# ikmb/vcf2prot

Hardware: AMD Instinct MI355X
Metric: amino-acids written/sec (higher is better)
Workload: dtype u8

## Files before the change

vcf2prot_amd/_native.py:

```python
from __future__ import annotations

import ctypes
import os
from ctypes import POINTER, c_char_p, c_double, c_int, c_int64, c_size_t, c_uint8, c_uint32, c_uint64, c_void_p

_PKG = os.path.dirname(os.path.abspath(__file__))
HIP_LIB_PATH = os.path.join(_PKG, "lib", "libvcf2prot_hip.so")
COHORT_LIB_PATH = os.path.join(_PKG, "lib", "libv2p_cohort.so")

V2P_OK = 0
ERR_NAMES = {
    0: "V2P_OK", -1: "V2P_ERR_INVALID_ARG", -2: "V2P_ERR_HIP", -3: "V2P_ERR_BAD_CODE", -4: "V2P_ERR_RES_OOB",
    -5: "V2P_ERR_SRC_OOB", -6: "V2P_ERR_NOT_CONTIGUOUS", -7: "V2P_ERR_NOT_CANONICAL", -8: "V2P_ERR_NON_BYTE_CHAR",
    -9: "V2P_ERR_UNSUPPORTED", -10: "V2P_ERR_STATE",
}
V2P_ERR_INVALID_ARG, V2P_ERR_HIP, V2P_ERR_BAD_CODE, V2P_ERR_RES_OOB, V2P_ERR_SRC_OOB = -1, -2, -3, -4, -5
V2P_ERR_NOT_CONTIGUOUS, V2P_ERR_NOT_CANONICAL, V2P_ERR_NON_BYTE_CHAR, V2P_ERR_UNSUPPORTED, V2P_ERR_STATE = -6, -7, -8, -9, -10
V2P_FLAG_DEBUG_GPU, V2P_FLAG_TEMPORAL, V2P_FLAG_RESULT_ORDER = 1, 2, 4


class v2p_chunk(ctypes.Structure):
    _fields_ = [("task_begin", c_uint64), ("dst_n", c_uint64)]


# ... 123 lines not shown

def hip_lib():
    global _hip
    if _hip is None:
        if not os.path.exists(HIP_LIB_PATH):
            raise RuntimeError(
                f"{HIP_LIB_PATH} is missing: build it with `python -m vcf2prot_amd.build` "
                "(the gpu engine has no CPU fallback)")
        _hip = _bind(ctypes.CDLL(HIP_LIB_PATH), HIP_API)
    return _hip


BENCH_LIB_PATH = os.path.join(_PKG, "lib", "libv2p_bench.so")
BENCH_API = {
    "v2p_copy_prefetch_launch": (c_int, [c_void_p, c_void_p, c_uint64, c_uint32, c_void_p, c_uint64, c_int, c_int, c_uint32]),
    "v2p_copy_mix_launch": (c_int, [c_void_p, c_void_p, c_uint64, c_uint32, c_void_p, c_uint64, c_void_p, c_uint32, c_uint32, c_uint32, c_uint32]),
    "v2p_copy_bench_launch": (c_int, [c_void_p, c_void_p, c_uint64, c_uint32, c_void_p, c_uint64, c_int, c_void_p]),
    "v2p_gather_bench_launch": (c_int, [c_void_p, c_void_p, c_uint64, c_uint32, c_uint32, c_uint32, c_void_p]),
    "v2p_fill_launch": (c_int, [c_void_p, c_void_p, c_uint64, c_uint32, c_int]),
    "v2p_stitch_launch": (c_int, [c_void_p, c_void_p, c_uint64, c_void_p, c_uint32, c_void_p, c_uint64, c_void_p, c_uint64,
                                  c_void_p, c_uint64, c_void_p, c_int, c_uint32]),
    "v2p_batch_download_patch_image": (c_int, [c_void_p, c_void_p, c_void_p, c_void_p, POINTER(c_uint64), POINTER(c_uint64)]),
    "v2p_bench_set_variant": (c_int, [c_void_p, c_uint32]),
    "v2p_scan_launch": (c_int, [c_void_p, c_int, c_void_p, c_uint64, c_void_p, c_void_p]),
}
_bench = None


def bench_lib():
    global _bench
    if _bench is None:
        if not os.path.exists(BENCH_LIB_PATH):
            from . import build
            build.build_bench()
        _bench = _bind(_bind(ctypes.CDLL(BENCH_LIB_PATH), HIP_API), BENCH_API)
    return _bench


def cohort_lib():
    global _cohort
    if _cohort is None:
        if not os.path.exists(COHORT_LIB_PATH):
            raise RuntimeError(f"{COHORT_LIB_PATH} is missing: build it with `python -m vcf2prot_amd.build`")
        from ._cohort_api import COHORT_API
        _cohort = _bind(ctypes.CDLL(COHORT_LIB_PATH), COHORT_API)
    return _cohort
# ... 9 lines not shown
```

vcf2prot_amd/csrc/stitch_device.hpp:

```cpp
#pragma once
#include <hip/hip_runtime.h>
#include <stdint.h>
#include "stitch_kernels.h"
#include "block_scan.hpp"

namespace v2p {

typedef uint32_t u32x4 __attribute__((ext_vector_type(4)));
struct __attribute__((packed, aligned(1))) unaligned16 { u32x4 v; };

__device__ __forceinline__ u32x4 gather16(uint64_t addr)
{
    typedef const __attribute__((address_space(1))) unaligned16* gptr;
    return reinterpret_cast<gptr>(addr)->v;
}

struct __attribute__((packed, aligned(4))) dwaligned16 { u32x4 v; };
__device__ __forceinline__ u32x4 gather16_dw(uint64_t addr)
{
    typedef const __attribute__((address_space(1))) dwaligned16* gptr;
    typedef const __attribute__((address_space(1))) uint32_t* dptr;
    const uint64_t base = addr & ~3ull;
    const uint32_t sh = uint32_t(addr) & 3u;
    const u32x4 v = reinterpret_cast<gptr>(base)->v;
// ... 42 lines not shown
    else if (q < 8) { lo = x; hi = y; }
    else { lo = 0ull; hi = x; }
    return u32x4{uint32_t(lo), uint32_t(lo >> 32), uint32_t(hi), uint32_t(hi >> 32)};
}

constexpr uint64_t ADJ_IMM = 1ull << 63;
constexpr uint64_t ADJ_LIT = (1ull << 40) - 1;

__device__ __forceinline__ void report(unsigned long long* status, uint64_t index, uint32_t reason)
{
    atomicMin(status, (unsigned long long)((index << 8) | reason));
}

__device__ __forceinline__ void lds_barrier()
{
    asm volatile("s_waitcnt lgkmcnt(0)" ::: "memory");
    __builtin_amdgcn_s_barrier();
    asm volatile("" ::: "memory");
}


__device__ __forceinline__ uint32_t touch_wave_first(uint32_t r, uint32_t q) { return r + 8u * 4u * q; }
__host__ __device__ __forceinline__ uint32_t touch_waves_per_xcd(uint32_t n_chunks) { return ((n_chunks + 7u) / 8u + 3u) / 4u; }
constexpr uint32_t STAGE_SLOTS = 64;
constexpr uint32_t TOUCH_CHUNKS_PER_WAVE = 4;
__device__ __forceinline__ void touch_chunks(const uint64_t* __restrict__ desc, const Chunk* __restrict__ chunks, uint32_t c0, uint32_t n_chunks, uint64_t n_desc,
                                             const uint8_t* __restrict__ payload, uint64_t payload_len, uint32_t lane, uint64_t* __restrict__ stage = nullptr,
                                             const uint64_t* __restrict__ rows = nullptr)
{
    if (c0 >= n_chunks) return;
    auto payload_lines = [&](uint64_t dd) {
        const uint64_t src = dd & SRC_MASK, len = (dd >> 40) & LEN_MASK;
        if ((dd >> 62) == SPACE_PAYLOAD && len != 0u && src < payload_len && len <= payload_len - src) {
            const uint32_t b0 = payload[src], b1 = payload[src + len - 1u];
            asm volatile("" :: "v"(b0), "v"(b1));
        }
    };
    if (rows) {
        uint64_t r[TOUCH_CHUNKS_PER_WAVE], t[TOUCH_CHUNKS_PER_WAVE];
#pragma unroll
        for (uint32_t k = 0; k < TOUCH_CHUNKS_PER_WAVE; ++k) {
            const uint32_t c = c0 + 8u * k < n_chunks ? c0 + 8u * k : c0;
            r[k] = rows[uint64_t(c) * STAGE_SLOTS + lane];
            t[k] = reinterpret_cast<const uint64_t*>(chunks + c)[lane & 1u];
        }
#pragma unroll
// ... 34 lines not shown
```

vcf2prot_amd/csrc/stitch_kernels.h:

```cpp
#pragma once
#include <hip/hip_runtime.h>
#include <stdint.h>
#include "sir_pack.hpp"

namespace v2p {

enum : uint32_t {
    STATUS_BAD_CODE = 1,
    STATUS_RES_OOB = 2,
    STATUS_SRC_OOB = 3,
    STATUS_NOT_CONTIGUOUS = 4
};
constexpr unsigned long long STATUS_CLEAN = ~0ull;
constexpr int STITCH_TASKS_PER_LANE = 4;
constexpr uint32_t DOTS_BYTES = 64u * 1024u + 128u;

struct StitchArgs {
    const uint64_t* desc;
    uint64_t        n_desc;
    const Chunk*    chunks;
    uint32_t        n_chunks;
    const uint8_t*  src0;
    uint64_t        src0_len;
    const uint8_t*  src1;
// ... 2 lines not shown
    uint64_t        out_len;
    unsigned long long* status;
    const uint8_t*  dots;
    const Chunk*    next_chunks = nullptr;
    uint32_t        n_next = 0;
    uint32_t        store_sc1 = 0;
    uint64_t        opt_phase_bytes = 0;
    uint32_t        opt_phase_min_chunks = 0;
    int32_t         opt_store_sc1 = -1;
    uint32_t        opt_touch = 0;
    uint32_t        opt_wave_bodies = 0;
    uint32_t        rows = 0;
    uint64_t        img_desc = 0, img_bytes = 0;
    hipStream_t     aux_stream = nullptr;
    hipEvent_t      ev_fork = nullptr, ev_join = nullptr;
    uint32_t        opt_dual = 0;
    uint64_t*       stage = nullptr;
    uint32_t        stage_chunks = 0;
    const uint64_t* stage_cur = nullptr;
    uint64_t*       stage_next = nullptr;
    const uint64_t* resident = nullptr;
    const uint64_t* rows_next = nullptr;
    uint32_t        phase_chunks = 0;
};

uint32_t stitch_stage_chunks(const StitchArgs& args, int nontemporal);
hipError_t launch_stage_rows(const StitchArgs& args, uint64_t* rows, hipStream_t stream);

struct OrderedArgs {
    const uint8_t*  code;
    const uint64_t* start_pos;
    const uint64_t* length;
    const uint64_t* start_pos_res;
    uint64_t        n_tasks;
    const uint8_t*  ref;
    const uint8_t*  alt;
    uint8_t*        res;
    uint64_t        esize;
};

struct ValidateArgs {
    const uint8_t*  code;
    const uint64_t* start_pos;
    const uint64_t* length;
    const uint64_t* start_pos_res;
    uint64_t        n_tasks;
    uint64_t        n_ref, n_alt, n_res;
// ... 25 lines not shown
```

vcf2prot_amd/csrc/stitch_kernels.hip:

```cpp
#include <hip/hip_runtime.h>
#include <utility>
#include <vector>
#include <stdint.h>
#include <stdlib.h>
#include <mutex>
#include "stitch_kernels.h"
#include "stitch_device.hpp"

namespace v2p {

__device__ __forceinline__ u32x4 overwrite_tail(u32x4 v, u32x4 ld, uint32_t ja, bool take)
{
    const uint64_t x = ~0ull << (8u * (ja & 7u));
    const uint64_t mlo = (take && ja < 8u) ? x : 0ull;
    const uint64_t mhi = take ? (ja < 8u ? ~0ull : x) : 0ull;
    const uint32_t k0 = uint32_t(mlo), k1 = uint32_t(mlo >> 32), k2 = uint32_t(mhi), k3 = uint32_t(mhi >> 32);
    v[0] = (v[0] & ~k0) | (ld[0] & k0);
    v[1] = (v[1] & ~k1) | (ld[1] & k1);
    v[2] = (v[2] & ~k2) | (ld[2] & k2);
    v[3] = (v[3] & ~k3) | (ld[3] & k3);
    return v;
}

template <bool DW>
// ... 1041 lines not shown
{
    if (blockIdx.x < n) rows[(first + blockIdx.x) * STAGE_SLOTS + threadIdx.x] = uint64_t(SPACE_FILL) << 62;
}

hipError_t launch_stage_rows(const StitchArgs& a, uint64_t* rows, hipStream_t stream)
{
    if (a.n_chunks == 0 || !rows) return hipSuccess;
    hipLaunchKernelGGL(touch_image_kernel, dim3(8u * ((touch_waves_per_xcd(a.n_chunks) + 3u) / 4u)), dim3(256), 0, stream, a.desc, a.chunks, a.n_chunks, a.n_desc, a.src1, a.src1_len, rows, nullptr);
    const uint32_t pad = (8u - (a.n_chunks & 7u)) & 7u;
    if (pad) hipLaunchKernelGGL(fill_rows_kernel, dim3(pad), dim3(64), 0, stream, rows, uint64_t(a.n_chunks), pad);
    return hipGetLastError();
}

static hipError_t launch_stitch_range(const StitchArgs& args, hipStream_t stream, int nontemporal, uint32_t max_blocks);

#ifdef V2P_BENCH_VARIANTS
__global__ void idle_kernel(uint32_t us)
{
    const uint64_t t0 = __builtin_readcyclecounter();
    while (__builtin_readcyclecounter() - t0 < uint64_t(us) * 100u) __builtin_amdgcn_s_sleep(64);
}
#endif

static uint64_t phase_plan(const StitchArgs& a, int nontemporal, uint32_t max_blocks, bool staged, bool* ride_out)
{
    *ride_out = false;
    if (a.n_chunks == 0) return 0;
    const uint64_t img_desc = a.img_desc ? a.img_desc : a.n_desc, img_bytes = a.img_bytes ? a.img_bytes : a.out_len;
    const bool rich = image_is_rich(img_desc, img_bytes);
    uint64_t phase_bytes = rich ? PHASE_BYTES_RICH : PHASE_BYTES_DEFAULT;
    if (staged && rich && a.src0_len <= PHASE_STAGED_SMALL_REF) phase_bytes = PHASE_BYTES_STAGED;
    if (a.opt_phase_bytes == ~0ull) phase_bytes = 0;
    else if (a.opt_phase_bytes != 0) phase_bytes = a.opt_phase_bytes;
    const bool streams = (nontemporal & 4) != 0 || (nontemporal & 16) == 0;
    const uint32_t min_chunks = a.opt_phase_min_chunks ? a.opt_phase_min_chunks : PHASE_MIN_CHUNKS;
    if (max_blocks != 0 || phase_bytes == 0 || !streams || a.n_chunks < min_chunks) return 0;
    const double per_chunk = 16.0 + 8.0 * double(img_desc) / double(a.n_chunks);
    uint64_t per = uint64_t(double(phase_bytes) / per_chunk);
    const uint64_t per_min = a.opt_phase_min_chunks ? 8u : 4096u;
    per = per < per_min ? per_min : (per & ~7ull);
    const bool no_touch = (a.opt_touch & 1u) != 0, own_touch = (a.opt_touch & 2u) != 0;
    *ride_out = !own_touch && !no_touch && (nontemporal & 4) != 0 && (nontemporal & 48) == 48 && !(nontemporal & 2);
    return per;
}

uint32_t stitch_stage_chunks(const StitchArgs& args, int nontemporal)
{
    bool ride = false;
    const uint64_t per = phase_plan(args, nontemporal, 0, true, &ride);
    const int wsel = (nontemporal >> 28) & 3;
    if (!ride || !(nontemporal & 8) || wsel != 0 || (args.opt_touch & 4u) != 0 || args.opt_dual || per == 0 || per > 0x7FFFFFFFull) return 0;
    return uint32_t(per < args.n_chunks ? per : ((uint64_t(args.n_chunks) + 7u) & ~7ull));
}

hipError_t launch_stitch(const StitchArgs& args, hipStream_t stream, int nontemporal, uint32_t max_blocks)
{
    if (args.n_chunks == 0) return hipSuccess;
    StitchArgs a = args;
    hipError_t err = hipSuccess;
    a.dots = device_dots(&err);
    if (!a.dots) return err;
    a.rows = (nontemporal & 8) != 0;
    const uint64_t img_desc = a.img_desc ? a.img_desc : a.n_desc, img_bytes = a.img_bytes ? a.img_bytes : a.out_len;
    const bool rich = image_is_rich(img_desc, img_bytes);
    a.store_sc1 = a.opt_store_sc1 >= 0 ? uint32_t(a.opt_store_sc1 != 0) : uint32_t(!rich);
    bool ride = false;
    const uint64_t per = phase_plan(a, nontemporal, max_blocks, (args.stage != nullptr || args.resident != nullptr) && a.rows, &ride);
    if (per == 0) return launch_stitch_range(a, stream, nontemporal, max_blocks);
    const bool no_touch = (a.opt_touch & 1u) != 0;
    const int wsel = (nontemporal >> 28) & 3;
    if (ride && wsel == 0 && (a.opt_touch & 4u) != 0 && per <= 0x7FFFFFFFull) {
        const uint32_t n0 = uint32_t(args.n_chunks < per ? args.n_chunks : per);
        hipLaunchKernelGGL(touch_image_kernel, dim3(8u * ((touch_waves_per_xcd(n0) + 3u) / 4u)), dim3(256), 0, stream, a.desc, a.chunks, n0, a.n_desc, a.src1, a.src1_len, nullptr);
        a.phase_chunks = uint32_t(per);
        return launch_stitch_range(a, stream, nontemporal, 0);
    }
    if (ride && wsel == 0 && a.opt_dual && a.aux_stream && a.ev_fork && a.ev_join && args.n_chunks >= 4u * per) {
        const uint64_t half = (per / 2u) & ~7ull;
        std::vector<std::pair<uint64_t, uint32_t>> pieces;
        for (uint64_t c0 = 0; c0 < args.n_chunks; ) {
            uint64_t nc = pieces.size() == 1u ? (half / 2u) & ~7ull : half;
            if (nc == 0u) nc = 8u;
            if (nc > args.n_chunks - c0) nc = args.n_chunks - c0;
            pieces.emplace_back(c0, uint32_t(nc));
            c0 += nc;
        }
        err = hipEventRecord(a.ev_fork, stream);
        if (err == hipSuccess) err = hipStreamWaitEvent(a.aux_stream, a.ev_fork, 0);
        if (err != hipSuccess) return err;
        for (size_t i = 0; i < pieces.size(); ++i) {
            hipStream_t s = (i & 1u) ? a.aux_stream : stream;
            a.chunks = args.chunks + pieces[i].first;
            a.n_chunks = pieces[i].second;
            a.next_chunks = nullptr; a.n_next = 0;
            if (i + 2u < pieces.size()) { a.next_chunks = args.chunks + pieces[i + 2u].first; a.n_next = pieces[i + 2u].second; }
            if (i < 2u) hipLaunchKernelGGL(touch_image_kernel, dim3(8u * ((touch_waves_per_xcd(a.n_chunks) + 3u) / 4u)), dim3(256), 0, s, a.desc, a.chunks, a.n_chunks, a.n_desc, a.src1, a.src1_len, nullptr);
            err = launch_stitch_range(a, s, nontemporal, 0);
            if (err != hipSuccess) return err;
        }
        err = hipEventRecord(a.ev_join, a.aux_stream);
        if (err == hipSuccess) err = hipStreamWaitEvent(stream, a.ev_join, 0);
        return err != hipSuccess ? err : hipGetLastError();
    }
    const bool resident = ride && a.rows && wsel == 0 && args.resident != nullptr;
    const bool staged = !resident && ride && a.rows && wsel == 0 && args.stage != nullptr && per <= args.stage_chunks;
    uint32_t phase = 0;
    for (uint64_t c0 = 0; c0 < args.n_chunks; c0 += per, ++phase) {
        const uint32_t nc = uint32_t(args.n_chunks - c0 < per ? args.n_chunks - c0 : per);
        a.chunks = args.chunks + c0;
        a.n_chunks = nc;
        a.next_chunks = nullptr; a.n_next = 0;
        if (ride && c0 + per < args.n_chunks) {
            a.next_chunks = args.chunks + c0 + per;
            a.n_next = uint32_t(args.n_chunks - (c0 + per) < per ? args.n_chunks - (c0 + per) : per);
        }
        a.stage_cur = nullptr; a.stage_next = nullptr; a.rows_next = nullptr;
        if (resident) {
            a.stage_cur = args.resident + c0 * STAGE_SLOTS;
            if (a.next_chunks) a.rows_next = args.resident + (c0 + per) * STAGE_SLOTS;
        } else if (staged) {
            a.stage_cur = args.stage + uint64_t(phase & 1u) * args.stage_chunks * STAGE_SLOTS;
            a.stage_next = args.stage + uint64_t((phase + 1u) & 1u) * args.stage_chunks * STAGE_SLOTS;
        }
        if (!no_touch && (!ride || c0 == 0)) hipLaunchKernelGGL(touch_image_kernel, dim3(8u * ((touch_waves_per_xcd(nc) + 3u) / 4u)), dim3(256), 0, stream, a.desc, a.chunks, nc, a.n_desc, a.src1, a.src1_len,
                                                                 staged ? const_cast<uint64_t*>(a.stage_cur) : nullptr, resident ? a.stage_cur : nullptr);
        err = launch_stitch_range(a, stream, nontemporal, 0);
        if (err != hipSuccess) return err;
#ifdef V2P_BENCH_VARIANTS
// ... 136 lines not shown
```

vcf2prot_amd/csrc/stitch_wave.hip:

```cpp
#include <hip/hip_runtime.h>
#include <stdint.h>
#include <stdlib.h>
#include "stitch_kernels.h"
#include "stitch_device.hpp"

namespace v2p {

struct __attribute__((aligned(16))) WRec {
    uint32_t a_lo, a_hi;
    uint32_t se;
    uint32_t lit;
};
constexpr uint32_t WREC_NOLIT = 0xFFFFu;

__device__ __forceinline__ uint64_t wrec_adj(const WRec& t) { return (uint64_t(t.a_hi) << 32) | t.a_lo; }

__device__ __forceinline__ u32x4 put_byte(u32x4 v, uint32_t q, uint32_t byte)
{
    const uint32_t sh = 8u * (q & 3u), m = 0xFFu << sh, bv = byte << sh, k = q >> 2;
    v[0] = k == 0u ? (v[0] & ~m) | bv : v[0];
    v[1] = k == 1u ? (v[1] & ~m) | bv : v[1];
    v[2] = k == 2u ? (v[2] & ~m) | bv : v[2];
    v[3] = k == 3u ? (v[3] & ~m) | bv : v[3];
    return v;
// ... 40 lines not shown
constexpr uint32_t WAVE_ND = (WAVE_ROWS + 3u) / 4u;
struct WaveLds {
    uint32_t map32[64u * WAVE_ND];
    WRec rec[CHUNK_TASKS_WAVE + 4];
    u32x4 patch[CHUNK_TASKS_WAVE + 1];
};

template <uint32_t R, bool NT, bool SC1>
__device__ __forceinline__ void wave_rows(WaveLds& L, const u32x4* s_mask, const u32x4* s_one, const uint32_t lane, const uint32_t n, const uint32_t head,
                                          const uint32_t ptotal, const uint32_t nblk, const uint64_t dst, uint8_t* __restrict__ p_out, const uint64_t dots16,
                                          const uint64_t g1_addr, const WChk& chk);

#ifndef V2P_WAVE_OCC
#define V2P_WAVE_OCC 8
#endif
template <int WPG, bool NT, bool SC1 = false, bool RIMG = false, bool STG = false, int BODIES = 0>
__global__ __launch_bounds__(64 * WPG, V2P_WAVE_OCC) void stitchw_kernel(const uint64_t* __restrict__ p_desc, const Chunk* __restrict__ p_chunks,
                                                            const uint8_t* __restrict__ p_src0, const uint8_t* __restrict__ p_src1,
                                                            uint8_t* __restrict__ p_out, unsigned long long* __restrict__ p_status,
                                                            const uint8_t* __restrict__ p_dots,
                                                            uint32_t n_chunks, uint64_t n_desc, uint64_t src0_len, uint64_t src1_len, uint64_t out_len,
                                                            const Chunk* __restrict__ p_next, uint32_t n_next, uint32_t phase_chunks,
                                                            const uint64_t* __restrict__ p_stage = nullptr, uint64_t* __restrict__ p_stage_next = nullptr,
                                                            const uint64_t* __restrict__ p_rows_next = nullptr)
{
    static_assert(!STG || (RIMG && WPG == 1), "staged descriptors: rows images, one wave per workgroup");
    __shared__ __attribute__((aligned(16))) WaveLds s_all[WPG];
    __shared__ u32x4 s_mask[17];
    __shared__ u32x4 s_one[17];

    const uint32_t lane = threadIdx.x & 63u;
    const uint32_t wid = WPG == 1 ? 0u : uint32_t(__builtin_amdgcn_readfirstlane(int(threadIdx.x >> 6)));
    uint32_t c = blockIdx.x * uint32_t(WPG) + wid;
    if (WPG == 1 && phase_chunks != 0u) {
        const uint32_t tw = 8u * touch_waves_per_xcd(phase_chunks), per = tw + phase_chunks;
        const uint32_t g = blockIdx.x / per, r = blockIdx.x - g * per;
        if (r < tw) {
            const uint64_t base = uint64_t(g + 1u) * phase_chunks;
            if (base < n_chunks)
                touch_chunks(p_desc, p_chunks + base, touch_wave_first(r & 7u, r >> 3), uint32_t(n_chunks - base < phase_chunks ? n_chunks - base : phase_chunks),
                             n_desc, p_src1, src1_len, lane);
            return;
        }
        c = g * phase_chunks + (r - tw);
        if (c >= n_chunks) return;
    } else if (c >= n_chunks) {
        const uint32_t first_wg = (((n_chunks + uint32_t(WPG) - 1u) / uint32_t(WPG)) + 7u) & ~7u;
        if (blockIdx.x >= first_wg) {
            uint32_t q = ((blockIdx.x - first_wg) >> 3) * uint32_t(WPG) + wid;
            if (STG && p_rows_next) { const uint32_t tq = touch_waves_per_xcd(n_next); q = q < tq ? tq - 1u - q : q; }
            touch_chunks(p_desc, p_next, touch_wave_first(blockIdx.x & 7u, q), n_next, n_desc, p_src1, src1_len, lane,
                         STG ? p_stage_next : nullptr, STG ? p_rows_next : nullptr);
        }
        return;
    }
    WaveLds& L = s_all[wid];
    uint64_t d_stg = 0ull;
// ... 214 lines not shown
    if (lane < 2u) {
        const uint32_t b16 = lane == 0u ? 0u : (nblk - 1u) << 4;
        if ((b16 < head || b16 + 16u > ptotal) && (lane == 0u || b16 != 0u)) {
            const uint32_t hi = b16 + 16u < ptotal ? b16 + 16u : ptotal;
            uint32_t r = uint32_t(map8[b16 >> 4]);
            WRec t = L.rec[r];
            u32x4 o = wgather(wrec_adj(t) + b16, chk, 6u);
            o = wrec_lit(o, t.lit, b16);
            while ((t.se >> 16) < hi) {
                t = L.rec[++r];
                const u32x4 g = wgather(wrec_adj(t) + b16, chk, 7u);
                o = wmerge(o, g, s_mask[(t.se & 0xFFFFu) - b16]);
                o = wrec_lit(o, t.lit, b16);
            }
            const uint32_t ka = b16 < head ? head - b16 : 0u, kb = hi - b16;
            for (uint32_t q = ka; q < kb; ++q) out0[b16 + q] = uint8_t(o[q >> 2] >> (8u * (q & 3u)));
        }
    }
}

hipError_t launch_stitch_wave(const StitchArgs& a, hipStream_t stream, bool nt, int waves_per_group)
{
    if (a.n_chunks == 0) return hipSuccess;
    if (a.phase_chunks != 0u && waves_per_group == 1) {
        const uint32_t P = a.phase_chunks, tw = 8u * touch_waves_per_xcd(P);
        const uint64_t groups = (uint64_t(a.n_chunks) + P - 1u) / P, grid = groups * (uint64_t(tw) + P);
        if (grid > 0x7FFFFFFFull) return hipErrorInvalidValue;
        if (a.rows) {
            if (nt) hipLaunchKernelGGL((stitchw_kernel<1, true, false, true>), dim3(uint32_t(grid)), dim3(64), 0, stream, a.desc, a.chunks, a.src0, a.src1, a.out, a.status, a.dots,
                                       a.n_chunks, a.n_desc, a.src0_len, a.src1_len, a.out_len, nullptr, 0u, P);
            else hipLaunchKernelGGL((stitchw_kernel<1, false, false, true>), dim3(uint32_t(grid)), dim3(64), 0, stream, a.desc, a.chunks, a.src0, a.src1, a.out, a.status, a.dots,
                                    a.n_chunks, a.n_desc, a.src0_len, a.src1_len, a.out_len, nullptr, 0u, P);
            return hipGetLastError();
        }
        if (nt) hipLaunchKernelGGL((stitchw_kernel<1, true>), dim3(uint32_t(grid)), dim3(64), 0, stream, a.desc, a.chunks, a.src0, a.src1, a.out, a.status, a.dots,
                                   a.n_chunks, a.n_desc, a.src0_len, a.src1_len, a.out_len, nullptr, 0u, P);
        else hipLaunchKernelGGL((stitchw_kernel<1, false>), dim3(uint32_t(grid)), dim3(64), 0, stream, a.desc, a.chunks, a.src0, a.src1, a.out, a.status, a.dots,
                                a.n_chunks, a.n_desc, a.src0_len, a.src1_len, a.out_len, nullptr, 0u, P);
        return hipGetLastError();
    }
    uint32_t sub = 0;
#ifdef V2P_BENCH_VARIANTS
    if (const char* e = getenv("V2P_WAVE_SUB")) sub = uint32_t(strtoul(e, nullptr, 10));
#endif
    if (sub == 0 || sub > a.n_chunks) sub = a.n_chunks;
    sub = (sub + 7u) & ~7u;
// ... 25 lines not shown
        } else if (a.rows) { if (nt && a.store_sc1) V2P_LWR(true, true); else if (nt) V2P_LWR(true, false); else V2P_LWR(false, false); }
#ifdef V2P_BENCH_VARIANTS
        else if (waves_per_group == 4) { if (nt) V2P_LW(4, true); else V2P_LW(4, false); }
        else if (waves_per_group == 2) { if (nt) V2P_LW(2, true); else V2P_LW(2, false); }
#endif
        else if (nt && a.store_sc1) hipLaunchKernelGGL((stitchw_kernel<1, true, true>), dim3(tw ? (((nc + 7u) & ~7u) + 8u * tw) : nc), dim3(64), 0, stream,
                                                      a.desc, ch, a.src0, a.src1, a.out, a.status, a.dots, nc, a.n_desc, a.src0_len, a.src1_len, a.out_len, a.next_chunks, n_next, 0u);
        else { if (nt) V2P_LW(1, true); else V2P_LW(1, false); }
#undef V2P_LW
#undef V2P_LWR
#undef V2P_LWS
    }
    return hipGetLastError();
}

__global__ void code_object_loader_b() {}
hipError_t preload_stitch_wave(hipStream_t stream)
{
    hipLaunchKernelGGL(code_object_loader_b, dim3(1), dim3(64), 0, stream);
    return hipGetLastError();
}

}
```

vcf2prot_amd/csrc/v2p_api.hip:

```cpp
#include <hip/hip_runtime.h>
#include <cstdint>
#include <cstdio>
#include <cstring>
#include <atomic>
#include <chrono>
#include <condition_variable>
#include <cstdlib>
#include <functional>
#include <memory>
#include <mutex>
#include <new>
#include <string>
#include <thread>
#include <vector>

#include "../../include/vcf2prot_hip.h"
#include "sir_pack.hpp"
#include "stitch_kernels.h"
#include "build_kernels.h"
#include "build_rows.h"
#include "dense_pieces.h"
#ifdef V2P_BENCH_VARIANTS
#include "patch_image.h"
#include "bench/v2p_bench.h"
// ... 2112 lines not shown
        if (!fb) { stream_attach(b, st); return V2P_OK; }
        if (kernel == 9) return c->fail(V2P_ERR_UNSUPPORTED, "the stream does not fit a tile image: kernel 0 or 7 builds a dense rows image");
        mode = ROWS_DENSE;
    }
    int rc = build_rows_image(b, st->v, mode, build_ms, false);
    if (rc == V2P_ERR_UNSUPPORTED && kernel == 0 && mode == ROWS_WAVE) rc = build_rows_image(b, st->v, ROWS_DENSE, build_ms, false);
    if (rc == V2P_OK) stream_attach(b, st);
    return rc;
}

#ifdef V2P_BENCH_VARIANTS
static hipError_t patch_execute(v2p_batch* b, hipStream_t stream)
{
    v2p_ctx* c = b->ctx;
    PatchExecArgs a{reinterpret_cast<const uint64_t*>(b->d_desc.ptr()), reinterpret_cast<const uint32_t*>(b->d_patch.ptr()), reinterpret_cast<const Chunk*>(b->d_chunks.ptr()),
                    uint32_t(b->n_chunks), c->proteome.ptr(), c->proteome_len + c->headers_len, b->payload_dev, b->n_payload,
                    b->d_out.ptr(), b->out_bytes, reinterpret_cast<unsigned long long*>(b->d_status.ptr())};
    return launch_stitch_patch(a, stream, !(c->flags & V2P_FLAG_TEMPORAL));
}
#endif

static uint32_t touch_of(uint32_t variant) { return variant == 16u ? 4u : (variant == 17u ? 2u : (variant == 18u ? 1u : 0u)); }
static uint32_t wave_bodies_of(uint32_t variant) { return variant == 32u ? 1u : (variant == 33u ? 2u : 0u); }

static void dual_of(v2p_ctx* c, StitchArgs& a)
{
    if (ctx_variant(c) != 19u) return;
    if (!c->exec_aux && hipStreamCreateWithFlags(&c->exec_aux, hipStreamNonBlocking) != hipSuccess) { c->exec_aux = nullptr; return; }
    for (hipEvent_t& e : c->ev_exec) if (!e && hipEventCreateWithFlags(&e, hipEventDisableTiming) != hipSuccess) { e = nullptr; return; }
    a.aux_stream = c->exec_aux; a.ev_fork = c->ev_exec[0]; a.ev_join = c->ev_exec[1]; a.opt_dual = 1u;
}

static hipError_t ensure_event(hipEvent_t& e) { return e ? hipSuccess : hipEventCreate(&e); }


static bool stage_rich(const StitchArgs& a, bool small_ref)
{
    const uint64_t idesc = a.img_desc ? a.img_desc : a.n_desc, ibytes = a.img_bytes ? a.img_bytes : a.out_len;
    const uint64_t phase = a.opt_phase_bytes != 0 && a.opt_phase_bytes != ~0ull ? a.opt_phase_bytes : PHASE_BYTES_RICH;
    return image_is_rich(idesc, ibytes) && (!small_ref || a.src0_len <= PHASE_STAGED_SMALL_REF) && 8u * idesc + 16u * uint64_t(a.n_chunks) >= 8u * phase;
}

static hipError_t attach_stage(v2p_batch* b, StitchArgs& a, int hint)
{
    const bool small_rich = stage_rich(a, true);
    if (ctx_variant(b->ctx) == 23u || !(b->pad_image || ctx_variant(b->ctx) == 25u || small_rich)) return hipSuccess;
    const uint32_t rows = stitch_stage_chunks(a, hint);
    if (rows == 0) return hipSuccess;
    const hipError_t e = b->d_stage.ensure(uint64_t(2) * rows * 64u * 8u);
    if (e != hipSuccess) { (void)hipGetLastError(); return hipSuccess; }
    a.stage = reinterpret_cast<uint64_t*>(b->d_stage.ptr()); a.stage_chunks = rows;
    return hipSuccess;
}

static bool rows_wanted(const v2p_batch* b, const StitchArgs& a, int hint)
{
    const uint32_t var = ctx_variant(b->ctx);
    if (var == 23u || var == 30u || b->pad_image || b->is_tiles || b->is_patch) return false;
    return (stage_rich(a, false) || var == 31u) && stitch_stage_chunks(a, hint) != 0;
}

static bool attach_rows(v2p_batch* b, StitchArgs& a, int hint, hipError_t* err)
{
    *err = hipSuccess;
    if (!rows_wanted(b, a, hint) || b->rows_state < 0) return false;
    if (b->rows_state == 0) {
        const uint64_t n_rows = (b->n_chunks + 7u) & ~7ull;
        if (b->d_rows.ensure_exact(n_rows * uint64_t(CHUNK_TASKS_WAVE) * 8u) != hipSuccess) { (void)hipGetLastError(); b->rows_state = -1; return false; }
        *err = launch_stage_rows(a, reinterpret_cast<uint64_t*>(b->d_rows.ptr()), b->ctx->stream);
        if (*err == hipSuccess) *err = hipStreamSynchronize(b->ctx->stream);
        if (*err != hipSuccess) return false;
        b->rows_state = 1;
    }
    a.resident = reinterpret_cast<const uint64_t*>(b->d_rows.ptr());
    return true;
}

static hipError_t stitch_range(v2p_batch* b, uint64_t desc_bound, uint64_t chunk0, uint64_t n_chunks, uint64_t img_desc, uint64_t img_bytes, hipStream_t stream)
{
    v2p_ctx* c = b->ctx;
    if (n_chunks == 0) return hipSuccess;
    StitchArgs a{reinterpret_cast<const uint64_t*>(b->d_desc.ptr()), desc_bound, reinterpret_cast<const Chunk*>(b->d_chunks.ptr()) + chunk0,
// ... 581 lines not shown
    unsigned long long stw = ~0ull;
    HIP_TRY(c, hipMemcpyAsync(&total, basebuf.ptr() + nc * 8, 8, hipMemcpyDeviceToHost, c->stream), "D2H(pieces)");
    HIP_TRY(c, hipMemcpyAsync(&stw, st.ptr(), 8, hipMemcpyDeviceToHost, c->stream), "D2H(status)");
    HIP_TRY(c, hipStreamSynchronize(c->stream), "hipStreamSynchronize");
    if (stw != ~0ull || total == 0 || total >= (1ull << 40)) return V2P_OK;
    if (b->d_pieces.ensure(total * 8) != hipSuccess || b->d_chunks2.ensure(nc * sizeof(Chunk)) != hipSuccess) { (void)hipGetLastError(); return V2P_OK; }
    b->n_pieces = total; b->pieces_src0_len = a.src0_len; b->pieces_src1_len = a.src1_len;
    a.pieces = reinterpret_cast<uint64_t*>(b->d_pieces.ptr()); a.chunks2 = reinterpret_cast<Chunk*>(b->d_chunks2.ptr());
    HIP_TRY(c, launch_pieces_build(a, 1, c->stream), "launch(pieces: write)");
    HIP_TRY(c, hipStreamSynchronize(c->stream), "hipStreamSynchronize");
    b->pieces_state = 1;
    return V2P_OK;
}

static StitchArgs whole_table_args(const v2p_batch* b)
{
    const v2p_ctx* c = b->ctx;
    StitchArgs a{reinterpret_cast<const uint64_t*>(b->d_desc.ptr()), b->pad_image ? b->desc_slots : b->n_desc, reinterpret_cast<const Chunk*>(b->d_chunks.ptr()),
                 uint32_t(b->n_chunks), c->proteome.ptr(), c->proteome_len + c->headers_len, b->payload_dev, b->n_payload,
                 b->d_out.ptr(), b->out_bytes, reinterpret_cast<unsigned long long*>(b->d_status.ptr())};
    a.opt_phase_bytes = c->launch_opts.phase_bytes; a.opt_phase_min_chunks = c->launch_opts.phase_min_chunks; a.opt_store_sc1 = c->launch_opts.store_sc1;
    a.opt_touch = touch_of(ctx_variant(c));
    a.opt_wave_bodies = wave_bodies_of(ctx_variant(c));
    a.img_desc = b->pad_image ? b->n_desc : 0;
    return a;
}

int v2p_batch_execute(v2p_batch* b)
{
    if (!b) return V2P_ERR_INVALID_ARG;
    v2p_ctx* c = b->ctx;
    std::lock_guard<std::mutex> lk(c->mu);
    if (!b->finalized) return c->fail(V2P_ERR_STATE, "batch not finalized");
    if (b->orphaned) return c->fail(V2P_ERR_STATE, "the v2p_stream this batch was built from has been destroyed: its image cannot be executed again (the arena stays readable)");
    HIP_TRY(c, hipSetDevice(c->device), "hipSetDevice");
#ifdef V2P_BENCH_VARIANTS
    if (b->is_patch) {
        const hipError_t pe = patch_execute(b, c->stream);
        if (pe != hipSuccess) return c->hip_fail(pe, "launch(stitch: patch image)");
        return V2P_OK;
    }
#endif
    if (b->is_tiles) {
        if (c->proteome_len + c->headers_len < b->pieces_src0_len) return c->fail(V2P_ERR_SRC_OOB, "the resident reference is shorter than the one this tile image was built against: rebuild the batch");
        HIP_TRY(c, tiles_execute(b, c->stream), "launch(stitch: tile image)");
        b->executed = true;
// ... 36 lines not shown
    if (rc) (void)hipMemsetAsync(b->d_status.ptr(), 0xFF, sizeof(unsigned long long), c->stream);
    return rc;
}

int v2p_batch_counts(const v2p_batch* b, uint64_t* n_haps, uint64_t* n_desc, uint64_t* n_chunks,
                     uint64_t* out_bytes, uint64_t* payload_bytes)
{
    if (!b) return V2P_ERR_INVALID_ARG;
    std::lock_guard<std::mutex> lk(b->ctx->mu);
    const bool f = b->finalized;
    if (n_haps) *n_haps = f ? b->n_haps : b->img.n_haplotypes();
    if (n_desc) *n_desc = f ? b->n_desc : b->img.desc.size();
    if (n_chunks) *n_chunks = f ? b->n_chunks : b->img.chunks.size();
    if (out_bytes) *out_bytes = f ? b->out_bytes : b->img.out_size();
    if (payload_bytes) *payload_bytes = f ? b->n_payload : b->img.payload.size();
    return V2P_OK;
}

int v2p_batch_image_form(const v2p_batch* b)
{
    if (!b) return V2P_ERR_INVALID_ARG;
    std::lock_guard<std::mutex> lk(b->ctx->mu);
    bool resident = false;
    if (b->finalized && b->executed && b->rows_state == 1 && b->d_rows.ptr()) {
        StitchArgs a = whole_table_args(b);
        a.opt_dual = ctx_variant(b->ctx) == 19u ? 1u : 0u;
        resident = rows_wanted(b, a, int(!(b->ctx->flags & V2P_FLAG_TEMPORAL)) | b->launch_hint);
    }
    return (b->pad_image ? 1 : 0) | (b->pieces_state == 1 ? 2 : 0) | (b->d_stage.ptr() ? 4 : 0) | (b->is_tiles ? 8 : 0) | (resident ? 16 : 0);
}

int v2p_batch_hap_range(const v2p_batch* b, uint64_t h, uint64_t* begin, uint64_t* len)
{
    if (!b || !begin || !len) return V2P_ERR_INVALID_ARG;
    std::lock_guard<std::mutex> lk(b->ctx->mu);
    const std::vector<uint64_t>& hb = b->img.hap_out_begin;
    if (h + 1 >= hb.size()) return V2P_ERR_INVALID_ARG;
    *begin = hb[h]; *len = hb[h + 1] - hb[h];
    return V2P_OK;
}

int v2p_batch_download(v2p_batch* b, uint64_t begin, uint64_t len, uint8_t* out)
{
    if (!b || (len && !out)) return V2P_ERR_INVALID_ARG;
    v2p_ctx* c = b->ctx;
    std::lock_guard<std::mutex> lk(c->mu);
    if (!b->finalized) return c->fail(V2P_ERR_STATE, "batch not finalized");
    if (begin + len > b->out_bytes) return c->fail(V2P_ERR_INVALID_ARG, "range outside the arena");
    HIP_TRY(c, hipSetDevice(c->device), "hipSetDevice");
    if (len) HIP_TRY(c, hipMemcpyAsync(out, b->d_out.ptr() + begin, len, hipMemcpyDeviceToHost, c->stream), "D2H(out)");
    HIP_TRY(c, hipStreamSynchronize(c->stream), "hipStreamSynchronize");
    return V2P_OK;
// ... 622 lines not shown
```

vcf2prot_amd/engine.py:

```python
from __future__ import annotations

import ctypes
import enum
import os
from dataclasses import dataclass
from typing import Dict, List, Optional, Sequence, Tuple

import numpy as np

from . import _native as N
from ._native import V2PError


class Engine(enum.Enum):
    ST = 0
    MT = 1
    GPU = 2

    @staticmethod
    def from_str(name: str) -> "Engine":
        out = ctypes.c_int(-1)
        rc = N.hip_lib().v2p_engine_from_str(name.encode(), ctypes.byref(out))
        if rc != N.V2P_OK:
            raise ValueError(f"{name} is not a supported engine")
# ... 318 lines not shown

    def finalize(self):
        self.ctx._check(self._lib.v2p_batch_finalize(self._h))

    def build_on_device(self, stream, window_bytes: int, kernel: int = 2) -> float:
        ms = ctypes.c_float(0.0)
        self.ctx._check(self._lib.v2p_batch_build_on_device(self._h, ctypes.byref(stream.struct), window_bytes, kernel, ctypes.byref(ms)))
        return float(ms.value)

    def build_from_stream(self, rs: "ResidentStream", kernel: int = 0) -> float:
        ms = ctypes.c_float(0.0)
        self.ctx._check(self._lib.v2p_batch_build_from_stream(self._h, rs._h, kernel, ctypes.byref(ms)))
        self._stream_ref = rs
        return float(ms.value)

    def build_and_execute(self, rs: "ResidentStream", kernel: int = 0, n_slices: int = 0):
        self.ctx._check(self._lib.v2p_batch_build_and_execute(self._h, rs._h, kernel, n_slices))
        self._stream_ref = rs

    def image_form(self) -> dict:
        f = self._lib.v2p_batch_image_form(self._h)
        if f < 0:
            self.ctx._check(f)
        return {"padded": bool(f & 1), "pieces": bool(f & 2), "staging_buffers": bool(f & 4), "tiles": bool(f & 8), "resident_rows": bool(f & 16)}

    def oneshot_info(self) -> dict:
        info = N.OneShotInfo()
        self.ctx._check(self._lib.v2p_batch_oneshot_info(self._h, ctypes.byref(info)))
        return {"kernel": int(info.kernel), "n_slices": int(info.n_slices), "total_ms": float(info.total_ms), "build_ms": float(info.build_ms),
                "call_wall_ms": float(info.call_wall_ms), "tables_ms": float(info.tables_ms), "slice_build_ms": [float(info.slice_build_ms[j]) for j in range(int(info.n_slices))]}

    def reset(self):
        self.ctx._check(self._lib.v2p_batch_reset(self._h))

    def download_patch_image(self):
        n = self.counts()["n_chunks"]
        seg = np.zeros((n, 1024), dtype=np.uint64)
        patch = np.zeros((n, 1024), dtype=np.uint32)
        chunks = np.zeros((n, 2), dtype=np.uint64)
        ns, npat = ctypes.c_uint64(), ctypes.c_uint64()
        self.ctx._check(self._lib.v2p_batch_download_patch_image(self._h, seg.ctypes.data if n else None, patch.ctypes.data if n else None,
                                                                 chunks.ctypes.data if n else None, ctypes.byref(ns), ctypes.byref(npat)))
        return seg, patch, chunks, int(ns.value), int(npat.value)

    def download_image(self):
        cn = self.counts()
        n_haps, n_desc, n_chunks = cn["n_haps"], cn["n_desc"], cn["n_chunks"]
# ... 168 lines not shown
```

Baseline: 5104 billion.

## Group multiple resident-row phases per stitch launch with interleaved read-ahead touch waves

When descriptor rows are resident, the stitch now packs several phases (four by default) into one kernel launch instead of one launch per phase. Each group's block range holds the phase's stitch waves plus touch waves that prefetch the next phase, inserted at a configurable offset, with a standalone touch kernel only before the first group. This cuts per-phase launch overhead and boundary bubbles. The cost is a more complex block-to-work mapping and touches that may be issued too early or too late relative to the stitch waves.

```diff
diff --git a/vcf2prot_amd/_native.py b/vcf2prot_amd/_native.py
--- a/vcf2prot_amd/_native.py
+++ b/vcf2prot_amd/_native.py
@@ -169,6 +169,7 @@
                                   c_void_p, c_uint64, c_void_p, c_int, c_uint32]),
     "v2p_batch_download_patch_image": (c_int, [c_void_p, c_void_p, c_void_p, c_void_p, POINTER(c_uint64), POINTER(c_uint64)]),
     "v2p_bench_set_variant": (c_int, [c_void_p, c_uint32]),
+    "v2p_bench_phase_map": (c_uint64, [c_uint32, c_uint32, c_uint32, c_uint32, c_uint32, c_uint32, c_uint32, c_void_p]),
     "v2p_scan_launch": (c_int, [c_void_p, c_int, c_void_p, c_uint64, c_void_p, c_void_p]),
 }
 _bench = None
diff --git a/vcf2prot_amd/csrc/stitch_device.hpp b/vcf2prot_amd/csrc/stitch_device.hpp
--- a/vcf2prot_amd/csrc/stitch_device.hpp
+++ b/vcf2prot_amd/csrc/stitch_device.hpp
@@ -88,6 +88,21 @@
 
 __device__ __forceinline__ uint32_t touch_wave_first(uint32_t r, uint32_t q) { return r + 8u * 4u * q; }
 __host__ __device__ __forceinline__ uint32_t touch_waves_per_xcd(uint32_t n_chunks) { return ((n_chunks + 7u) / 8u + 3u) / 4u; }
+struct PhaseSlot { uint32_t phase, read_ahead, index; };
+__host__ __device__ __forceinline__ PhaseSlot phase_group_slot(uint32_t b, uint32_t per, uint32_t tw, uint32_t at)
+{
+    const uint32_t span = per + tw, g = b / span, r = b - g * span;
+    if (r >= at && r - at < tw) return PhaseSlot{g, 1u, r - at};
+    return PhaseSlot{g, 0u, r < at ? r : r - tw};
+}
+__host__ __device__ __forceinline__ uint64_t phase_group_grid(uint32_t phases, uint32_t n_last, uint32_t n_next, uint32_t per, uint32_t tw, uint32_t at)
+{
+    const uint32_t stitch_end = n_last <= at ? n_last : n_last + tw;
+    const uint32_t read_end = n_next ? at + 8u * touch_waves_per_xcd(n_next) : 0u;
+    return uint64_t(phases - 1u) * (per + tw) + (stitch_end > read_end ? stitch_end : read_end);
+}
+constexpr uint32_t GROUP_AT_LAUNCH_ORDER = 0x80000000u;
+
 constexpr uint32_t STAGE_SLOTS = 64;
 constexpr uint32_t TOUCH_CHUNKS_PER_WAVE = 4;
 __device__ __forceinline__ void touch_chunks(const uint64_t* __restrict__ desc, const Chunk* __restrict__ chunks, uint32_t c0, uint32_t n_chunks, uint64_t n_desc,
diff --git a/vcf2prot_amd/csrc/stitch_kernels.h b/vcf2prot_amd/csrc/stitch_kernels.h
--- a/vcf2prot_amd/csrc/stitch_kernels.h
+++ b/vcf2prot_amd/csrc/stitch_kernels.h
@@ -48,7 +48,11 @@
     const uint64_t* resident = nullptr;
     const uint64_t* rows_next = nullptr;
     uint32_t        phase_chunks = 0;
+    uint32_t        group_at = 0;
+    uint32_t        opt_groups = 0;
 };
+
+uint32_t stitch_phase_groups(const StitchArgs& args, int nontemporal);
 
 uint32_t stitch_stage_chunks(const StitchArgs& args, int nontemporal);
 hipError_t launch_stage_rows(const StitchArgs& args, uint64_t* rows, hipStream_t stream);
diff --git a/vcf2prot_amd/csrc/stitch_kernels.hip b/vcf2prot_amd/csrc/stitch_kernels.hip
--- a/vcf2prot_amd/csrc/stitch_kernels.hip
+++ b/vcf2prot_amd/csrc/stitch_kernels.hip
@@ -1087,7 +1087,16 @@
 }
 #endif
 
-static uint64_t phase_plan(const StitchArgs& a, int nontemporal, uint32_t max_blocks, bool staged, bool* ride_out)
+struct PhaseGroups {
+    uint32_t G = 1u;
+    uint32_t at = 0u;
+    bool launch_order = false;
+    bool one_per_launch(uint64_t per) const { return G == 1u && at == per && !launch_order; }
+};
+constexpr uint32_t PHASE_GROUPS_ALL = 0x7FFFFFFFu;
+constexpr uint32_t PHASE_GROUP_DEFAULT = 4u;
+
+static uint64_t phase_plan(const StitchArgs& a, int nontemporal, uint32_t max_blocks, bool staged, bool* ride_out, PhaseGroups* groups = nullptr)
 {
     *ride_out = false;
     if (a.n_chunks == 0) return 0;
@@ -1106,6 +1115,19 @@
     per = per < per_min ? per_min : (per & ~7ull);
     const bool no_touch = (a.opt_touch & 1u) != 0, own_touch = (a.opt_touch & 2u) != 0;
     *ride_out = !own_touch && !no_touch && (nontemporal & 4) != 0 && (nontemporal & 48) == 48 && !(nontemporal & 2);
+    if (groups) {
+        PhaseGroups g;
+        g.G = PHASE_GROUP_DEFAULT;
+        uint32_t eighths = 8u;
+        bool back8 = false;
+        if (a.opt_groups != 0u && a.opt_groups <= 60u) {
+            static const uint32_t Gs[5] = {1u, 2u, 4u, 8u, PHASE_GROUPS_ALL}, shares[6] = {8u, 7u, 6u, 4u, 0u, 8u};
+            const uint32_t v = (a.opt_groups - 1u) % 30u;
+            g.G = Gs[v % 5u]; eighths = shares[v / 5u]; back8 = v / 5u == 5u; g.launch_order = a.opt_groups > 30u;
+        }
+        g.at = uint32_t(((per > 0x7FFFFFFFull ? 0x7FFFFFF8ull : per) * eighths / 8u) & ~7ull) - (back8 && per >= 8u ? 8u : 0u);
+        *groups = g;
+    }
     return per;
 }
 
@@ -1116,6 +1138,16 @@
     const int wsel = (nontemporal >> 28) & 3;
     if (!ride || !(nontemporal & 8) || wsel != 0 || (args.opt_touch & 4u) != 0 || args.opt_dual || per == 0 || per > 0x7FFFFFFFull) return 0;
     return uint32_t(per < args.n_chunks ? per : ((uint64_t(args.n_chunks) + 7u) & ~7ull));
+}
+
+uint32_t stitch_phase_groups(const StitchArgs& args, int nontemporal)
+{
+    bool ride = false;
+    PhaseGroups g;
+    const uint64_t per = phase_plan(args, nontemporal, 0, true, &ride, &g);
+    if (stitch_stage_chunks(args, nontemporal) == 0 || g.one_per_launch(per)) return 0;
+    const uint64_t phases = (uint64_t(args.n_chunks) + per - 1u) / per;
+    return uint32_t(g.G < phases ? g.G : phases);
 }
 
 hipError_t launch_stitch(const StitchArgs& args, hipStream_t stream, int nontemporal, uint32_t max_blocks)
@@ -1130,7 +1162,8 @@
     const bool rich = image_is_rich(img_desc, img_bytes);
     a.store_sc1 = a.opt_store_sc1 >= 0 ? uint32_t(a.opt_store_sc1 != 0) : uint32_t(!rich);
     bool ride = false;
-    const uint64_t per = phase_plan(a, nontemporal, max_blocks, (args.stage != nullptr || args.resident != nullptr) && a.rows, &ride);
+    PhaseGroups grp;
+    const uint64_t per = phase_plan(a, nontemporal, max_blocks, (args.stage != nullptr || args.resident != nullptr) && a.rows, &ride, &grp);
     if (per == 0) return launch_stitch_range(a, stream, nontemporal, max_blocks);
     const bool no_touch = (a.opt_touch & 1u) != 0;
     const int wsel = (nontemporal >> 28) & 3;
@@ -1169,6 +1202,29 @@
     }
     const bool resident = ride && a.rows && wsel == 0 && args.resident != nullptr;
     const bool staged = !resident && ride && a.rows && wsel == 0 && args.stage != nullptr && per <= args.stage_chunks;
+    if (resident && per <= 0x7FFFFFFFull && !grp.one_per_launch(per)) {
+        const uint64_t phases = (uint64_t(args.n_chunks) + per - 1u) / per, span = per * (grp.G < phases ? grp.G : phases);
+        a.phase_chunks = uint32_t(per);
+        a.group_at = grp.at | (grp.launch_order ? GROUP_AT_LAUNCH_ORDER : 0u);
+        for (uint64_t c0 = 0; c0 < args.n_chunks; c0 += span) {
+            a.chunks = args.chunks + c0;
+            a.n_chunks = uint32_t(args.n_chunks - c0 < span ? args.n_chunks - c0 : span);
+            a.next_chunks = nullptr; a.n_next = 0; a.rows_next = nullptr; a.stage_next = nullptr;
+            a.stage_cur = args.resident + c0 * STAGE_SLOTS;
+            if (c0 + span < args.n_chunks) {
+                a.next_chunks = args.chunks + c0 + span;
+                a.n_next = uint32_t(args.n_chunks - (c0 + span) < per ? args.n_chunks - (c0 + span) : per);
+                a.rows_next = args.resident + (c0 + span) * STAGE_SLOTS;
+            }
+            if (c0 == 0) {
+                const uint32_t n0 = uint32_t(args.n_chunks < per ? args.n_chunks : per);
+                hipLaunchKernelGGL(touch_image_kernel, dim3(8u * ((touch_waves_per_xcd(n0) + 3u) / 4u)), dim3(256), 0, stream, a.desc, a.chunks, n0, a.n_desc, a.src1, a.src1_len, nullptr, a.stage_cur);
+            }
+            err = launch_stitch_range(a, stream, nontemporal, 0);
+            if (err != hipSuccess) return err;
+        }
+        return hipGetLastError();
+    }
     uint32_t phase = 0;
     for (uint64_t c0 = 0; c0 < args.n_chunks; c0 += per, ++phase) {
         const uint32_t nc = uint32_t(args.n_chunks - c0 < per ? args.n_chunks - c0 : per);
diff --git a/vcf2prot_amd/csrc/stitch_wave.hip b/vcf2prot_amd/csrc/stitch_wave.hip
--- a/vcf2prot_amd/csrc/stitch_wave.hip
+++ b/vcf2prot_amd/csrc/stitch_wave.hip
@@ -86,7 +86,7 @@
                                                             uint32_t n_chunks, uint64_t n_desc, uint64_t src0_len, uint64_t src1_len, uint64_t out_len,
                                                             const Chunk* __restrict__ p_next, uint32_t n_next, uint32_t phase_chunks,
                                                             const uint64_t* __restrict__ p_stage = nullptr, uint64_t* __restrict__ p_stage_next = nullptr,
-                                                            const uint64_t* __restrict__ p_rows_next = nullptr)
+                                                            const uint64_t* __restrict__ p_rows_next = nullptr, uint32_t group_at = 0u)
 {
     static_assert(!STG || (RIMG && WPG == 1), "staged descriptors: rows images, one wave per workgroup");
     __shared__ __attribute__((aligned(16))) WaveLds s_all[WPG];
@@ -96,7 +96,24 @@
     const uint32_t lane = threadIdx.x & 63u;
     const uint32_t wid = WPG == 1 ? 0u : uint32_t(__builtin_amdgcn_readfirstlane(int(threadIdx.x >> 6)));
     uint32_t c = blockIdx.x * uint32_t(WPG) + wid;
-    if (WPG == 1 && phase_chunks != 0u) {
+    if (STG && phase_chunks != 0u) {
+        const uint32_t at = group_at & ~GROUP_AT_LAUNCH_ORDER;
+        const PhaseSlot s = phase_group_slot(blockIdx.x, phase_chunks, 8u * touch_waves_per_xcd(phase_chunks), at);
+        const uint32_t base = (s.phase + s.read_ahead) * phase_chunks;
+        if (s.read_ahead) {
+            const bool inside = base < n_chunks;
+            const uint32_t n = inside ? (n_chunks - base < phase_chunks ? n_chunks - base : phase_chunks) : n_next;
+            const uint32_t tq = touch_waves_per_xcd(n);
+            uint32_t q = s.index >> 3;
+            if (q >= tq) return;
+            if (!(group_at & GROUP_AT_LAUNCH_ORDER)) q = tq - 1u - q;
+            touch_chunks(p_desc, inside ? p_chunks + base : p_next, touch_wave_first(blockIdx.x & 7u, q), n, n_desc, p_src1, src1_len, lane, nullptr,
+                         inside ? p_stage + uint64_t(base) * STAGE_SLOTS : p_rows_next);
+            return;
+        }
+        c = base + s.index;
+        if (c >= n_chunks) return;
+    } else if (WPG == 1 && phase_chunks != 0u) {
         const uint32_t tw = 8u * touch_waves_per_xcd(phase_chunks), per = tw + phase_chunks;
         const uint32_t g = blockIdx.x / per, r = blockIdx.x - g * per;
         if (r < tw) {
@@ -357,6 +374,18 @@
 hipError_t launch_stitch_wave(const StitchArgs& a, hipStream_t stream, bool nt, int waves_per_group)
 {
     if (a.n_chunks == 0) return hipSuccess;
+    if (a.phase_chunks != 0u && waves_per_group == 1 && a.rows && a.stage_cur) {
+        const uint32_t P = a.phase_chunks, tw = 8u * touch_waves_per_xcd(P), at = a.group_at & ~GROUP_AT_LAUNCH_ORDER;
+        if ((P & 7u) != 0u || (at & 7u) != 0u || at > P) return hipErrorInvalidValue;
+        const uint32_t phases = uint32_t((uint64_t(a.n_chunks) + P - 1u) / P), n_next = a.next_chunks && a.rows_next ? a.n_next : 0u;
+        const uint64_t grid = phase_group_grid(phases, a.n_chunks - (phases - 1u) * P, n_next, P, tw, at);
+        if (grid > 0x7FFFFFFFull) return hipErrorInvalidValue;
+#define V2P_LWG(NTT, SCC) hipLaunchKernelGGL((stitchw_kernel<1, NTT, SCC, true, true>), dim3(uint32_t(grid)), dim3(64), 0, stream, \
+        a.desc, a.chunks, a.src0, a.src1, a.out, a.status, a.dots, a.n_chunks, a.n_desc, a.src0_len, a.src1_len, a.out_len, a.next_chunks, n_next, P, a.stage_cur, nullptr, a.rows_next, a.group_at)
+        if (nt && a.store_sc1) V2P_LWG(true, true); else if (nt) V2P_LWG(true, false); else V2P_LWG(false, false);
+#undef V2P_LWG
+        return hipGetLastError();
+    }
     if (a.phase_chunks != 0u && waves_per_group == 1) {
         const uint32_t P = a.phase_chunks, tw = 8u * touch_waves_per_xcd(P);
         const uint64_t groups = (uint64_t(a.n_chunks) + P - 1u) / P, grid = groups * (uint64_t(tw) + P);
@@ -428,3 +457,16 @@
 }
 
 }
+
+#ifdef V2P_BENCH_VARIANTS
+#include "bench/v2p_bench.h"
+uint64_t v2p_bench_phase_map(uint32_t first, uint32_t count, uint32_t per, uint32_t at, uint32_t phases, uint32_t n_last, uint32_t n_next, uint32_t* out)
+{
+    const uint32_t tw = 8u * v2p::touch_waves_per_xcd(per);
+    for (uint32_t i = 0; out && i < count; ++i) {
+        const v2p::PhaseSlot s = v2p::phase_group_slot(first + i, per, tw, at);
+        out[3u * i] = s.phase; out[3u * i + 1u] = s.read_ahead; out[3u * i + 2u] = s.index;
+    }
+    return phases ? v2p::phase_group_grid(phases, n_last, n_next, per, tw, at) : 0ull;
+}
+#endif
diff --git a/vcf2prot_amd/csrc/v2p_api.hip b/vcf2prot_amd/csrc/v2p_api.hip
--- a/vcf2prot_amd/csrc/v2p_api.hip
+++ b/vcf2prot_amd/csrc/v2p_api.hip
@@ -2158,6 +2158,8 @@
 
 static uint32_t touch_of(uint32_t variant) { return variant == 16u ? 4u : (variant == 17u ? 2u : (variant == 18u ? 1u : 0u)); }
 static uint32_t wave_bodies_of(uint32_t variant) { return variant == 32u ? 1u : (variant == 33u ? 2u : 0u); }
+static uint32_t groups_of(uint32_t variant) { return variant >= 34u && variant < 154u ? (variant - 34u) % 60u + 1u : 0u; }
+static bool rows_for_all(uint32_t variant) { return variant == 31u || (variant >= 94u && variant < 154u); }
 
 static void dual_of(v2p_ctx* c, StitchArgs& a)
 {
@@ -2193,7 +2195,7 @@
 {
     const uint32_t var = ctx_variant(b->ctx);
     if (var == 23u || var == 30u || b->pad_image || b->is_tiles || b->is_patch) return false;
-    return (stage_rich(a, false) || var == 31u) && stitch_stage_chunks(a, hint) != 0;
+    return (stage_rich(a, false) || rows_for_all(var)) && stitch_stage_chunks(a, hint) != 0;
 }
 
 static bool attach_rows(v2p_batch* b, StitchArgs& a, int hint, hipError_t* err)
@@ -2821,6 +2823,7 @@
     a.opt_phase_bytes = c->launch_opts.phase_bytes; a.opt_phase_min_chunks = c->launch_opts.phase_min_chunks; a.opt_store_sc1 = c->launch_opts.store_sc1;
     a.opt_touch = touch_of(ctx_variant(c));
     a.opt_wave_bodies = wave_bodies_of(ctx_variant(c));
+    a.opt_groups = groups_of(ctx_variant(c));
     a.img_desc = b->pad_image ? b->n_desc : 0;
     return a;
 }
@@ -2903,12 +2906,15 @@
     if (!b) return V2P_ERR_INVALID_ARG;
     std::lock_guard<std::mutex> lk(b->ctx->mu);
     bool resident = false;
+    uint32_t groups = 0;
     if (b->finalized && b->executed && b->rows_state == 1 && b->d_rows.ptr()) {
         StitchArgs a = whole_table_args(b);
         a.opt_dual = ctx_variant(b->ctx) == 19u ? 1u : 0u;
-        resident = rows_wanted(b, a, int(!(b->ctx->flags & V2P_FLAG_TEMPORAL)) | b->launch_hint);
-    }
-    return (b->pad_image ? 1 : 0) | (b->pieces_state == 1 ? 2 : 0) | (b->d_stage.ptr() ? 4 : 0) | (b->is_tiles ? 8 : 0) | (resident ? 16 : 0);
+        const int hint = int(!(b->ctx->flags & V2P_FLAG_TEMPORAL)) | b->launch_hint;
+        resident = rows_wanted(b, a, hint);
+        if (resident) { groups = stitch_phase_groups(a, hint); if (groups > 0xFFFFu) groups = 0xFFFFu; }
+    }
+    return (b->pad_image ? 1 : 0) | (b->pieces_state == 1 ? 2 : 0) | (b->d_stage.ptr() ? 4 : 0) | (b->is_tiles ? 8 : 0) | (resident ? 16 : 0) | (groups ? 32 : 0) | int(groups << 8);
 }
 
 int v2p_batch_hap_range(const v2p_batch* b, uint64_t h, uint64_t* begin, uint64_t* len)
diff --git a/vcf2prot_amd/engine.py b/vcf2prot_amd/engine.py
--- a/vcf2prot_amd/engine.py
+++ b/vcf2prot_amd/engine.py
@@ -364,7 +364,8 @@
         f = self._lib.v2p_batch_image_form(self._h)
         if f < 0:
             self.ctx._check(f)
-        return {"padded": bool(f & 1), "pieces": bool(f & 2), "staging_buffers": bool(f & 4), "tiles": bool(f & 8), "resident_rows": bool(f & 16)}
+        return {"padded": bool(f & 1), "pieces": bool(f & 2), "staging_buffers": bool(f & 4), "tiles": bool(f & 8), "resident_rows": bool(f & 16),
+                "phase_groups": (f >> 8) & 0xFFFF if f & 32 else 0}
 
     def oneshot_info(self) -> dict:
         info = N.OneShotInfo()
```

Result: no change. 5132 billion, median of 6 (+0.6%).
